# AtharvBhat/otters

Measured on AMD Instinct MI355X. Metric: GB/s scanned + queries/sec, exact cosine top-10 over 10M x 768 f32 rows per GPU, higher is better.
Workload: dtype f32; 1 GPU; 10000000x768 f32 VecStore per GPU, single query, Metric::Cosine, take(10); rows_per_gpu=10000000, dim=768, k=10, nq=1, processes=1

## Files before the change

### otters_amd/csrc/ott_exact.hip

```cpp
#include <atomic>

#include "ott_internal.h"
#include "ott_prune.h"
#include "ott_i8_check.h"
#include "ott_exact_dev.h"

namespace ott {

constexpr int KC = 32;
constexpr int WAVES = 4;
constexpr int STAGE_FLOATS = 64 * KC;
constexpr int EXACT_SMEM = WAVES * STAGE_FLOATS * 4;
constexpr int DUMP_QCAP = 128;
constexpr int EXACT_SMEM_DUMP = EXACT_SMEM + WAVES * DUMP_QCAP * 12;
constexpr int PQ_CAP = 128;
constexpr int PQ_WORDS = 10;
constexpr int QD_WORDS = (int)(OTT_QEMB_MAX / KC) * 12;
constexpr int EXACT_SMEM_PRUNE = EXACT_SMEM + WAVES * PQ_CAP * PQ_WORDS * 4 + QD_WORDS * 4;
constexpr int Q8_WORDS = (int)((OTT_QEMB_MAX + 127) / 128) * 32;
constexpr int EXACT_SMEM_CHECK = EXACT_SMEM_PRUNE + Q8_WORDS * 4;
#ifdef OTT_SK4_DECODE_F32
constexpr bool SK4_INT = false;
#else
constexpr bool SK4_INT = true;
#endif
constexpr int SK_MAXW = (int)OTT_SKETCH1_MAX_WORDS;
constexpr int SK3_MAXST = (int)OTT_SKETCH_MAX_WORDS / 3;
constexpr int SK3_XP = ((int)OTT_SKETCH_MAX_WORDS + 2 + 3) / 4 - 8;
#ifndef OTT_X_BLOCKS_PER_CU
#define OTT_X_BLOCKS_PER_CU 2
#endif
constexpr int BLOCKS_PER_CU = OTT_X_BLOCKS_PER_CU;
constexpr int SMALL_RING = 8;
constexpr uint32_t SMALL_QMAX = 2048;
[[maybe_unused]] constexpr int EXACT_SMEM_SMALL = SMALL_RING * STAGE_FLOATS * 4 + SMALL_QMAX * 4;

__device__ __forceinline__ void exact_glds16(const char* sbase, uint32_t voff, uint32_t lds_addr) {
    uint32_t keep;
    lds_addr = (uint32_t)__builtin_amdgcn_readfirstlane((int)lds_addr);
    asm volatile(
        "s_nop 4\n\t"
        "s_mov_b32 %0, m0\n\t"
        "s_mov_b32 m0, %3\n\t"
        "s_nop 0\n\t"
        "global_load_lds_dwordx4 %1, %2\n\t"
        "s_mov_b32 m0, %0"
        : "=&s"(keep)
        : "v"(voff), "s"(sbase), "s"(lds_addr)
        : "memory");
}


template <int MK, int NQ, int E, bool PERQ, bool DUMP = false, bool SMALL = false, bool BLK = (E > 1), bool I8 = false, bool PRUNE = false, int SK = 0, bool SEED = false,
          bool CHK = false>
__global__ __launch_bounds__(SMALL ? 64 : 256) void exact_kernel(ExactParams p) {
    static_assert(!CHK || (SK == 5 && !SEED && E == 1), "the int8 check is the gated head launch's, one list entry per lane");
    static_assert(!I8 || (NQ == 1 && MK == MK_DOT && !PERQ && !DUMP && !SMALL), "the int8 sweep takes one query, cosine / dot, merged");
    static_assert(!PRUNE || (NQ == 1 && MK == MK_DOT && !PERQ && !DUMP && !SMALL && !I8), "the pruned sweep takes one query, cosine / dot, merged");
    static_assert((SK == 0 || PRUNE) && (SK == 0 || SK == 1 || SK == 3 || SK == 4 || SK == 5), "the sketch is the pruned sweep's: none, one, three or four bits per dim (5: four with a head)");
    constexpr bool HD = SK == 5;
    constexpr bool SK4 = SK == 4 || SK == 5;
    static_assert(!HD || SK4_INT, "the head form decodes by integer dot products only");
    static_assert(!SEED || (HD && E == 1), "the estimate pass is the head form's, one list entry per lane");
    extern __shared__ __attribute__((aligned(16))) float smem[];
    const int lane = threadIdx.x & 63;
    const int wave = __builtin_amdgcn_readfirstlane(threadIdx.x >> 6);
    constexpr int BW = SMALL ? 1 : WAVES;
    float* st = SMALL ? smem : smem + wave * STAGE_FLOATS;
    float* sQ = smem + SMALL_RING * STAGE_FLOATS;
    constexpr int NL = PERQ ? NQ : 1;
    constexpr int KS = 64 * E;

    WaveList<E> L[NL];
    uint64_t tk[NL];
    uint32_t tq[NL];
    bool fresh[NL];
#pragma unroll
    for (int i = 0; i < NL; i++) {
        wl_init(L[i]);
        tk[i] = 0;
        tq[i] = 0xFFFFFFFFu;
        fresh[i] = true;
    }

    const bool take_max = p.take_max != 0;
    const uint32_t nq_here = (p.nq_total - p.q0) < (uint32_t)NQ ? (p.nq_total - p.q0) : (uint32_t)NQ;
    typedef __attribute__((address_space(4))) const float* CF32;
    typedef __attribute__((address_space(4))) const uint32_t* CU32;
    typedef __attribute__((address_space(4))) const ott_run* CRUN;
    typedef __attribute__((address_space(4))) const char* CCH;
    const CCH karg = (CCH)__builtin_amdgcn_kernarg_segment_ptr();
    const CF32 Q = p.embedded ? (CF32)(karg + __builtin_offsetof(ExactParams, qemb)) : (CF32)(p.queries + (size_t)p.q0 * p.dimq);
    const CU32 tile_prefix = p.embedded ? (CU32)(karg + __builtin_offsetof(ExactParams, eprefix)) : (CU32)p.tile_prefix;
    const CRUN runs = p.embedded ? (CRUN)(karg + __builtin_offsetof(ExactParams, eruns)) : (CRUN)p.runs;
    float qinv[NQ];
#pragma unroll
    for (int q = 0; q < NQ; q++) qinv[q] = (uint32_t)q < nq_here ? (p.embedded ? p.eqinv : p.qinv[p.q0 + q]) : 0.0f;
    uint32_t dgate[NQ];
#pragma unroll
    for (int q = 0; q < NQ; q++) dgate[q] = (DUMP && p.dump_gate != nullptr && (uint32_t)q < nq_here) ? p.dump_gate[p.q0 + q] : 0u;
    uint64_t* dq_key = reinterpret_cast<uint64_t*>(smem + WAVES * STAGE_FLOATS) + wave * DUMP_QCAP;
    uint32_t* dq_q = reinterpret_cast<uint32_t*>(smem + WAVES * STAGE_FLOATS + WAVES * DUMP_QCAP * 2) + wave * DUMP_QCAP;
    uint32_t dqn = 0;
    auto dq_flush = [&]() {
        if (dqn == 0) return;
        wave_sync();
        unsigned long long base = 0;
        if (lane == 0) base = atomicAdd(p.dump_cursor, (unsigned long long)dqn);
        base = rl64(base, 0);
        for (uint32_t i = lane; i < dqn; i += 64) {
            const uint64_t at = base + i;
            if (at < p.dump_cap) {
                p.dump_keys[at] = dq_key[i];
                p.dump_q[at] = dq_q[i];
            }
        }
        wave_sync();
        dqn = 0;
    };

    if constexpr (SMALL) {
        for (uint32_t i = threadIdx.x; i < p.dimq; i += 64 * BW) sQ[i] = Q[i];
        __syncthreads();
    }
    const uint32_t gw = blockIdx.x * BW + wave, nw = gridDim.x * BW;
    const int sw = (lane >> 1) & 7;
    const uint32_t nstages = (p.ld + KC - 1) / KC;
    [[maybe_unused]] uint32_t* qd = reinterpret_cast<uint32_t*>(smem + WAVES * STAGE_FLOATS + WAVES * PQ_CAP * PQ_WORDS);
    [[maybe_unused]] uint32_t* q8w = qd + QD_WORDS;
    [[maybe_unused]] const uint32_t ld8w = ((p.dim + 127u) & ~127u) >> 2;
    if constexpr (CHK) {
        const float pf8 = p.metric == OTT_METRIC_COSINE ? qinv[0] : 1.0f;
        const float inv_sq = __fdiv_rn(1.0f, p.i8_qscale);
        const uint32_t nw8 = ld8w < (uint32_t)Q8_WORDS ? ld8w : (uint32_t)Q8_WORDS;
        for (uint32_t i = threadIdx.x; i < nw8; i += 64 * BW) {
            float q4[4];
#pragma unroll
            for (int j = 0; j < 4; j++) q4[j] = (4 * i + j < p.dim) ? Q[4 * i + j] : 0.0f;
            q8w[i] = i8_quant_word(q4, pf8, inv_sq);
        }
    }
    if constexpr (SK4 && SK4_INT) {
        const uint32_t nqs = nstages < (uint32_t)(QD_WORDS / 12) ? nstages : (uint32_t)(QD_WORDS / 12);
        for (uint32_t i = threadIdx.x; i < nqs * 4; i += 64 * BW) {
            float q8[8];
#pragma unroll
            for (int j = 0; j < 8; j++) q8[j] = (8 * i + j < p.dim) ? Q[8 * i + j] : 0.0f;
            uint32_t d3[3];
            prune_quant_word(q8, p.prune_qinv_scale, d3);
#pragma unroll
            for (int d = 0; d < 3; d++) qd[(i >> 2) * 12 + d * 4 + (i & 3)] = d3[d];
        }
        __syncthreads();
    }
    const int lrow = lane >> 3;
    const int lslot = lane & 7;
    const uint32_t lsl4 = ((uint32_t)lslot * 4 < p.ld) ? (uint32_t)lslot * 4 : 0u;

    const uint32_t pstage = HD ? 0u : p.prune_stage;
    const uint32_t s_end = PRUNE ? pstage : nstages;
    uint32_t theta = 0;
    if constexpr (PRUNE && !SEED) {
        if (p.prune_seed[0] >= p.k) theta = ord_of(reinterpret_cast<const ott_hit*>(p.prune_seed + 8)[p.k - 1].score, take_max);
    }
    float* pq = smem + WAVES * STAGE_FLOATS + wave * (PQ_CAP * PQ_WORDS);
    uint32_t* pq_row = reinterpret_cast<uint32_t*>(pq + 9 * PQ_CAP);
    uint32_t pq_head = 0, pq_n = 0;
    uint32_t tails_done = 0;
    auto pq_finish = [&](uint32_t n) {
        wave_sync();
        const bool valid = (uint32_t)lane < n;
        const uint32_t e = (pq_head + (valid ? (uint32_t)lane : 0u)) & (PQ_CAP - 1);
        float acc[8];
#pragma unroll
        for (int l = 0; l < 8; l++) acc[l] = pq[l * PQ_CAP + e];
        const float vinv = pq[8 * PQ_CAP + e];
        const uint32_t my_row = pq_row[e];
        float tail = 0.0f;
        const float* rp[8];
        bool rok[8];
#pragma unroll
        for (int m = 0; m < 8; m++) {
            const uint32_t i = 8 * m + lrow;
            rok[m] = i < n;
            rp[m] = p.rows + (uint64_t)pq_row[(pq_head + (rok[m] ? i : 0u)) & (PQ_CAP - 1)] * p.ld + lsl4;
        }
        v4f R[8];
        auto load_stage = [&](uint32_t s) {
            const uint32_t soff = (s * KC + lslot * 4 < p.ld) ? s * KC : 0u;
#pragma unroll
            for (int m = 0; m < 8; m++) R[m] = __builtin_nontemporal_load(reinterpret_cast<const v4f*>(rp[m] + soff));
        };
        load_stage(pstage);
        for (uint32_t s = pstage; s < nstages; s++) {
            const bool cok = s * KC + lslot * 4 < p.ld;
#pragma unroll
            for (int m = 0; m < 8; m++) {
                const int row = 8 * m + lrow;
                const bool ok = rok[m] & cok;
                const v4f v = R[m];
                *reinterpret_cast<float4*>(st + row * KC + ((lslot ^ ((row >> 1) & 7)) << 2)) =
                    make_float4(ok ? v.x : 0.f, ok ? v.y : 0.f, ok ? v.z : 0.f, ok ? v.w : 0.f);
            }
            wave_sync();
            if (s + 1 < nstages) load_stage(s + 1);
#pragma unroll
            for (int j = 0; j < KC / 8; j++) {
                const uint32_t col = s * KC + 8 * j;
                if (col < p.dim) {
                    const float4 a = *reinterpret_cast<const float4*>(st + lane * KC + (((2 * j) ^ sw) << 2));
                    const float4 b = *reinterpret_cast<const float4*>(st + lane * KC + (((2 * j + 1) ^ sw) << 2));
                    const float x[8] = {a.x, a.y, a.z, a.w, b.x, b.y, b.z, b.w};
                    if (col + 8 <= p.dim) {
#pragma unroll
                        for (int l = 0; l < 8; l++) acc[l] = __fadd_rn(acc[l], exact_term<MK>(Q[col + l], x[l]));
                    } else {
                        const uint32_t nt = p.dim - col;
#pragma unroll
                        for (int l = 0; l < 7; l++)
                            if ((uint32_t)l < nt) tail = __fadd_rn(tail, exact_term<MK>(Q[col + l], x[l]));
                    }
                }
            }
            wave_sync();
        }
        float sc = __fadd_rn(reduce8(acc, p.reduce), tail);
        if (p.metric == OTT_METRIC_COSINE) sc = __fmul_rn(__fmul_rn(sc, qinv[0]), vinv);
        const bool pass = valid && !(sc != sc) && cmp_holds(sc, p.cmp, p.thr);
        const uint64_t key = ((uint64_t)ord_of(sc, take_max) << 32) | (uint32_t)(~(my_row + p.tie_off));
        if (fresh[0]) {
            wl_fill_sorted(L[0], tk[0], tq[0], p.k, pass, key, p.q0, lane, p.tie_sh);
            fresh[0] = false;
        } else if constexpr (!BLK) {
            wl_offer(L[0], tk[0], tq[0], p.k, pass, key, p.q0, lane, p.tie_sh);
        } else {
            wl_offer_block(L[0], tk[0], tq[0], p.k, pass, key, p.q0, lane, p.tie_sh);
        }
        pq_head = (pq_head + n) & (PQ_CAP - 1);
        pq_n -= n;
        tails_done += n;
    };
    [[maybe_unused]] uint32_t queued = 0;
    [[maybe_unused]] auto pq_refine = [&](uint32_t n, uint32_t gate) __attribute__((always_inline)) -> uint32_t {
        typedef uint32_t v4u __attribute__((ext_vector_type(4)));
        wave_sync();
        const bool valid = (uint32_t)lane < n;
        const uint32_t e = (pq_head + (valid ? (uint32_t)lane : 0u)) & (PQ_CAP - 1);
        const float vinv = pq[8 * PQ_CAP + e];
        const uint32_t my_row = pq_row[e];
        const float sv = p.i8_scale[my_row];
        const uint32_t fl = p.flag[my_row];
        const uint32_t* rp[8];
#pragma unroll
        for (int m = 0; m < 8; m++) {
            const uint32_t i = 8 * m + lrow;
            rp[m] = reinterpret_cast<const uint32_t*>(p.chk_plane) + (uint64_t)pq_row[(pq_head + (i < n ? i : 0u)) & (PQ_CAP - 1)] * ld8w + (uint32_t)lslot * 4;
        }
        v4f R[8];
        auto load_stage = [&](uint32_t s) {
#pragma unroll
            for (int m = 0; m < 8; m++) R[m] = __builtin_nontemporal_load(reinterpret_cast<const v4f*>(rp[m] + s * KC));
        };
        const uint32_t nst8 = ld8w / KC;
        int iacc[2] = {0, 0};
        load_stage(0);
        for (uint32_t s = 0; s < nst8; s++) {
#pragma unroll
            for (int m = 0; m < 8; m++) {
                const int row = 8 * m + lrow;
                const v4f v = R[m];
                *reinterpret_cast<float4*>(st + row * KC + ((lslot ^ ((row >> 1) & 7)) << 2)) = make_float4(v.x, v.y, v.z, v.w);
            }
            wave_sync();
            if (s + 1 < nst8) load_stage(s + 1);
#pragma unroll
            for (int j = 0; j < KC / 8; j++) {
                const float4 a = *reinterpret_cast<const float4*>(st + lane * KC + (((2 * j) ^ sw) << 2));
                const float4 b = *reinterpret_cast<const float4*>(st + lane * KC + (((2 * j + 1) ^ sw) << 2));
                const int x[8] = {__float_as_int(a.x), __float_as_int(a.y), __float_as_int(a.z), __float_as_int(a.w),
                                  __float_as_int(b.x), __float_as_int(b.y), __float_as_int(b.z), __float_as_int(b.w)};
                const v4u* qp = reinterpret_cast<const v4u*>(q8w + s * KC + 8 * j);
                const v4u q0 = qp[0], q1 = qp[1];
#pragma unroll
                for (int l = 0; l < 4; l++) {
                    iacc[0] = __builtin_amdgcn_sdot4(x[l], (int)q0[l], iacc[0], false);
                    iacc[1] = __builtin_amdgcn_sdot4(x[4 + l], (int)q1[l], iacc[1], false);
                }
            }
            wave_sync();
        }
        const float approx = i8_approx_score(iacc[0] + iacc[1], i8_row_factor(p.metric == OTT_METRIC_COSINE, vinv, sv, p.i8_qscale));
        const bool stay = valid && !i8_check_drops(approx, p.chk_eps, take_max, gate, (fl & 5u) != 0);
        const uint64_t km = __ballot(stay);
        if (stay) {
            const uint32_t at = (pq_head + (uint32_t)__popcll(km & ((1ull << lane) - 1ull))) & (PQ_CAP - 1);
            pq[8 * PQ_CAP + at] = vinv;
            pq_row[at] = my_row;
        }
        return (uint32_t)__popcll(km);
    };
    [[maybe_unused]] auto pq_drain = [&](uint32_t n, uint32_t gate) __attribute__((always_inline)) {
        const uint32_t stay = gate != 0 ? pq_refine(n, gate) : n;
        if (stay) pq_finish(stay);
        pq_head = (pq_head + (n - stay)) & (PQ_CAP - 1);
        pq_n -= n - stay;
    };

    if constexpr (HD) {
        typedef uint32_t v4u __attribute__((ext_vector_type(4)));
        const uint32_t np = p.sk_pitch >> 2;
        auto locate = [&](uint32_t t, uint64_t& row0, uint32_t& cnt, uint64_t& vm) {
            uint32_t lo = 0, hi = p.n_runs;
            while (hi - lo > 1) {
                uint32_t mid = (lo + hi) >> 1;
                if (tile_prefix[mid] <= t) lo = mid;
                else hi = mid;
            }
            const uint64_t rs = runs[lo].start, rc = runs[lo].count;
            const uint64_t off = (uint64_t)(t - tile_prefix[lo]) * 64;
            row0 = rs + off;
            cnt = (rc - off) < 64 ? (uint32_t)(rc - off) : 64u;
            const uint64_t r = row0 + lane;
            bool valid = (uint32_t)lane < cnt;
            if (p.row_mask != nullptr && valid && r < p.row_mask_bits) valid = (p.row_mask[r >> 6] >> (r & 63)) & 1;
            vm = __ballot(valid);
        };
        auto next_tile = [&](uint32_t t, uint64_t& row0, uint32_t& cnt, uint64_t& vm) -> uint32_t {
            for (; t < p.n_tiles; t += nw) {
                locate(t, row0, cnt, vm);
                if (vm != 0) break;
            }
            return t;
        };
        v4f R[8];
        v4u hc = {0u, 0u, 0u, 0u};
        float hrho = __builtin_inff(), hinv = 0.0f;
        auto load_line = [&](uint64_t row0, uint32_t cnt, uint32_t f) {
            const uint32_t pc = (8 * f + (uint32_t)lslot < np) ? 8 * f + (uint32_t)lslot : np - 1;
            const uint32_t* lb = p.prune_sketch + row0 * (uint64_t)p.sk_pitch + 4 * pc;
#pragma unroll
            for (int m = 0; m < 8; m++) {
                const uint32_t row = 8 * m + lrow;
                R[m] = __builtin_nontemporal_load(reinterpret_cast<const v4f*>(lb + (row < cnt ? row : cnt - 1) * p.sk_pitch));
            }
        };
        auto load_head = [&](uint64_t row0, uint32_t cnt) {
            const uint64_t r = row0 + ((uint32_t)lane < cnt ? (uint32_t)lane : cnt - 1);
            hc = __builtin_nontemporal_load(reinterpret_cast<const v4u*>(p.prune_head_codes) + r);
            hrho = __builtin_nontemporal_load(p.prune_head_rho + r);
            hinv = __builtin_nontemporal_load(p.inv + r);
        };
        uint64_t row0 = 0, vm = 0;
        uint32_t cnt = 0;
        uint32_t t = next_tile(gw, row0, cnt, vm);
        bool pf = false;
        while (t < p.n_tiles) {
            uint32_t gate = theta;
            const uint32_t own = (uint32_t)(tk[0] >> 32);
            if (own > gate) gate = own;
            const uint64_t my_row = row0 + lane;
            const bool valid = (vm >> lane) & 1;
            uint64_t row0n = 0, vmn = 0;
            uint32_t cntn = 0;
            const uint32_t tn = next_tile(t + nw, row0n, cntn, vmn);
            bool keep = valid;
            float vinv = 0.0f;
            if (SEED || gate != 0) {
                if (!pf) {
                    load_line(row0, cnt, 0);
                    load_head(row0, cnt);
                }
                const v4u c0 = hc;
                const float rho_all = hrho;
                vinv = hinv;
                pf = false;
                int K0 = 0, K1 = 0, K2 = 0;
                float sk_a = 0.0f;
                for (uint32_t f = 0; 8 * f < np; f++) {
#pragma unroll
                    for (int m = 0; m < 8; m++) {
                        const int row = 8 * m + lrow;
                        const v4f v = R[m];
                        *reinterpret_cast<float4*>(st + row * KC + ((lslot ^ ((row >> 1) & 7)) << 2)) = make_float4(v.x, v.y, v.z, v.w);
                    }
                    wave_sync();
                    if (8 * (f + 1) < np) {
                        load_line(row0, cnt, f + 1);
                    } else if (tn < p.n_tiles) {
                        load_line(row0n, cntn, 0);
                        load_head(row0n, cntn);
                        pf = true;
                    }
                    for (uint32_t j = 0; j < 8 && 8 * f + j < np; j++) {
                        const float4 w4 = *reinterpret_cast<const float4*>(st + lane * KC + (((int)j ^ sw) << 2));
                        const uint32_t piece = 8 * f + j;
                        if (piece == 0) {
                            sk_a = w4.x;
                            continue;
                        }
                        const uint32_t sj = p.sk_stage0 + piece - 1u;
                        if (sj < nstages) {
                            const uint32_t w[4] = {__float_as_uint(w4.x), __float_as_uint(w4.y), __float_as_uint(w4.z), __float_as_uint(w4.w)};
                            const v4u* dp = reinterpret_cast<const v4u*>(qd + sj * 12);
                            const v4u d0 = dp[0], d1 = dp[1], d2 = dp[2];
#pragma unroll
                            for (int i = 0; i < 4; i++) {
                                K0 = __builtin_amdgcn_sdot8((int)w[i], (int)d0[i], K0, false);
                                K1 = __builtin_amdgcn_sdot8((int)w[i], (int)d1[i], K1, false);
                                K2 = __builtin_amdgcn_sdot8((int)w[i], (int)d2[i], K2, false);
                            }
                        }
                    }
                    wave_sync();
                }
                {
                    const v4u* dp = reinterpret_cast<const v4u*>(qd);
                    const v4u d0 = dp[0], d1 = dp[1], d2 = dp[2];
#pragma unroll
                    for (int i = 0; i < 4; i++) {
                        K0 = __builtin_amdgcn_sdot8((int)c0[i], (int)d0[i], K0, false);
                        K1 = __builtin_amdgcn_sdot8((int)c0[i], (int)d1[i], K1, false);
                        K2 = __builtin_amdgcn_sdot8((int)c0[i], (int)d2[i], K2, false);
                    }
                }
                if constexpr (SEED) {
                    const int K = 2 * (256 * K2 + 16 * K1 + K0) + p.prune_qsum;
                    const float est = prune_score_est_sketchq(vinv, sk_a, rho_all, K, p.prune_qscale, qinv[0], p.metric == OTT_METRIC_COSINE);
                    const bool offer = valid && est - est == 0.0f;
                    const uint64_t key = ((uint64_t)ord_of(est, take_max) << 32) | (uint32_t)(~(uint32_t)my_row);
                    if (fresh[0]) {
                        wl_fill_sorted(L[0], tk[0], tq[0], p.seed_keep, offer, key, p.q0, lane, 0u);
                        fresh[0] = false;
                    } else {
                        wl_offer(L[0], tk[0], tq[0], p.seed_keep, offer, key, p.q0, lane, 0u);
                    }
                    keep = false;
                } else if (valid) {
                    const float zero[8] = {0.f, 0.f, 0.f, 0.f, 0.f, 0.f, 0.f, 0.f};
                    const int K = 2 * (256 * K2 + 16 * K1 + K0) + p.prune_qsum;
                    const float b = prune_score_bound_sketchq(zero, vinv, sk_a, rho_all, K, p.prune_qscale, p.dim, p.prune_qt, p.prune_qe1, p.prune_qn, qinv[0],
                                                              p.metric == OTT_METRIC_COSINE, take_max);
                    keep = !(b == b && ord_of(b, take_max) < gate);
                }
            } else if (valid) {
                vinv = p.inv[my_row];
            }
            const uint64_t km = SEED ? 0ull : __ballot(keep);
            if (!SEED && keep) {
                const uint32_t at = (pq_head + pq_n + (uint32_t)__popcll(km & ((1ull << lane) - 1ull))) & (PQ_CAP - 1);
#pragma unroll
                for (int l = 0; l < 8; l++) pq[l * PQ_CAP + at] = 0.0f;
                pq[8 * PQ_CAP + at] = vinv;
                pq_row[at] = (uint32_t)my_row;
            }
            pq_n += (uint32_t)__popcll(km);
            if constexpr (CHK) queued += (uint32_t)__popcll(km);
            if (!SEED && pq_n >= 64) {
                if constexpr (CHK) pq_drain(64, gate);
                else pq_finish(64);
                if (pf) {
                    load_line(row0n, cntn, 0);
                    load_head(row0n, cntn);
                }
            }
            t = tn;
            row0 = row0n;
            cnt = cntn;
            vm = vmn;
        }
        if constexpr (SEED) {
            const bool have = (uint32_t)lane < p.seed_keep && L[0].key[0] != 0ull;
            const uint64_t hm = __ballot(have);
            if (have) {
                const uint32_t r = ~(uint32_t)L[0].key[0];
                const uint32_t at = (uint32_t)__popcll(hm & ((1ull << lane) - 1ull));
#pragma unroll
                for (int l = 0; l < 8; l++) pq[l * PQ_CAP + at] = 0.0f;
                pq[8 * PQ_CAP + at] = p.inv[r];
                pq_row[at] = r;
            }
            pq_n = (uint32_t)__popcll(hm);
            wl_init(L[0]);
            tk[0] = 0;
            tq[0] = 0xFFFFFFFFu;
            fresh[0] = true;
        }
    } else
    for (uint32_t t = gw; t < p.n_tiles; t += nw) {
        uint32_t lo = 0, hi = p.n_runs;
        while (hi - lo > 1) {
            uint32_t mid = (lo + hi) >> 1;
            if (tile_prefix[mid] <= t) lo = mid;
            else hi = mid;
        }
        ott_run run;
        run.start = runs[lo].start;
        run.count = runs[lo].count;
        const uint64_t off = (uint64_t)(t - tile_prefix[lo]) * 64;
        const uint64_t row0 = run.start + off;
        const uint32_t cnt = (run.count - off) < 64 ? (uint32_t)(run.count - off) : 64u;
        const uint64_t my_row = row0 + lane;
        bool valid = (uint32_t)lane < cnt;
        if (p.row_mask != nullptr && valid && my_row < p.row_mask_bits)
            valid = (p.row_mask[my_row >> 6] >> (my_row & 63)) & 1;
        if (__ballot(valid) == 0) continue;

        float vinv = 0.0f;
        if ((PRUNE || p.metric == OTT_METRIC_COSINE) && valid) vinv = p.inv[my_row];
        float vsq = 0.0f;
        typedef uint32_t v4u __attribute__((ext_vector_type(4)));
        [[maybe_unused]] uint32_t skl[2 + SK_MAXW];
        [[maybe_unused]] uint32_t gate3 = 0;
        if constexpr (SK >= 3) {
            gate3 = theta;
            const uint32_t own = (uint32_t)(tk[0] >> 32);
            if (own > gate3) gate3 = own;
        }
        if constexpr (SK == 1) {
#pragma unroll
            for (int i = 0; i < 2 + SK_MAXW; i++) skl[i] = 0u;
            skl[1] = 0x7F800000u;
            if (valid) {
                const v4u* sp = reinterpret_cast<const v4u*>(p.prune_sketch + my_row * (uint64_t)p.sk_pitch);
                const v4u l0 = __builtin_nontemporal_load(sp);
                v4u l1 = {0u, 0u, 0u, 0u}, l2 = {0u, 0u, 0u, 0u};
                if (p.sk_pitch > 4) l1 = __builtin_nontemporal_load(sp + 1);
                if (p.sk_pitch > 8) l2 = __builtin_nontemporal_load(sp + 2);
                skl[0] = l0.x; skl[1] = l0.y; skl[2] = l0.z; skl[3] = l0.w;
                skl[4] = l1.x; skl[5] = l1.y; skl[6] = l1.z; skl[7] = l1.w;
                skl[8] = l2.x; skl[9] = l2.y; skl[10] = l2.z; skl[11] = l2.w;
            }
        }
        float i8_rf = 0.0f;
        bool i8_forced = false;
        if constexpr (I8) {
            if (valid) {
                i8_rf = ((p.metric == OTT_METRIC_COSINE ? vinv : 1.0f) * p.i8_scale[my_row]) * p.i8_qscale;
                i8_forced = (p.flag[my_row] & 5u) != 0;
            }
        }
        int iacc[2] = {0, 0};
        float acc[NQ][8];
        float tail[NQ];
#pragma unroll
        for (int q = 0; q < NQ; q++) {
            tail[q] = 0.0f;
#pragma unroll
            for (int l = 0; l < 8; l++) acc[q][l] = 0.0f;
        }

        v4f R[8];
        const float* rp[8];
        bool rok[8];
        const uint32_t lds_ring = (uint32_t)(uintptr_t)(__attribute__((address_space(3))) void*)st;
        const char* dma_base = reinterpret_cast<const char*>(p.rows + row0 * (uint64_t)p.ld);
        uint32_t dma_row[8];
        if constexpr (SMALL) {
#pragma unroll
            for (int m = 0; m < 8; m++) {
                const uint32_t row = 8 * m + lrow;
                dma_row[m] = (row < cnt ? row : cnt - 1) * p.ld;
            }
        } else {
#pragma unroll
            for (int m = 0; m < 8; m++) {
                const uint32_t row = 8 * m + lrow;
                rok[m] = row < cnt;
                rp[m] = p.rows + (row0 + (rok[m] ? row : cnt - 1)) * (uint64_t)p.ld + lsl4;
            }
        }
        auto dma_stage = [&](uint32_t s) {
            const uint32_t slot_e = lslot ^ (lrow >> 1);
#pragma unroll
            for (int m = 0; m < 8; m++) {
                const uint32_t col = s * KC + ((m & 1) ? (slot_e ^ 4) : slot_e) * 4;
                exact_glds16(dma_base, (dma_row[m] + (col < p.ld ? col : 0u)) * 4u,
                             lds_ring + (uint32_t)((s % SMALL_RING) * STAGE_FLOATS * 4 + m * 1024));
            }
        };
        auto load_stage = [&](uint32_t s) {
            const uint32_t soff = (s * KC + lslot * 4 < p.ld) ? s * KC : 0u;
#pragma unroll
            for (int m = 0; m < 8; m++) {
                R[m] = __builtin_nontemporal_load(reinterpret_cast<const v4f*>(rp[m] + soff));
            }
        };

        auto load_line = [&](uint32_t f) {
            const uint32_t np = p.sk_pitch >> 2;
            const uint32_t pc = (8 * f + (uint32_t)lslot < np) ? 8 * f + (uint32_t)lslot : np - 1;
            const uint32_t* lb = p.prune_sketch + row0 * (uint64_t)p.sk_pitch + 4 * pc;
#pragma unroll
            for (int m = 0; m < 8; m++) {
                const uint32_t row = 8 * m + lrow;
                R[m] = __builtin_nontemporal_load(reinterpret_cast<const v4f*>(lb + (row < cnt ? row : cnt - 1) * p.sk_pitch));
            }
        };

        if constexpr (SMALL) {
            for (uint32_t s = 0; s < (uint32_t)(SMALL_RING - 1) && s < nstages; s++) dma_stage(s);
        } else {
            load_stage(0);
        }
        for (uint32_t s = 0; s < s_end; s++) {
            const float* sst = st;
            if constexpr (SMALL) {
                const uint32_t later = (nstages - 1 - s) < (uint32_t)(SMALL_RING - 2) ? (nstages - 1 - s) : (uint32_t)(SMALL_RING - 2);
                switch (later) {
                    case 0: asm volatile("s_waitcnt vmcnt(0)" ::: "memory"); break;
                    case 1: asm volatile("s_waitcnt vmcnt(8)" ::: "memory"); break;
                    case 2: asm volatile("s_waitcnt vmcnt(16)" ::: "memory"); break;
                    case 3: asm volatile("s_waitcnt vmcnt(24)" ::: "memory"); break;
// ... 134 lines not shown
                                    for (int b = 0; b < 32; b++) {
                                        const int code = (int)(w[b >> 3] << (28 - 4 * (b & 7))) >> 28;
                                        D = fmaf((float)(2 * code + 1), Q[sj * KC + b], D);
                                    }
                                }
                            }
                        }
                        wave_sync();
                    }
                    if (valid) {
                        float b;
                        if constexpr (SK4_INT) {
                            const int K = 2 * (256 * K2 + 16 * K1 + K0) + p.prune_qsum;
                            b = prune_score_bound_sketchq(acc[0], vinv, sk_a, sk_rho, K, p.prune_qscale, p.dim, p.prune_qt, p.prune_qe1, p.prune_qn, qinv[0],
                                                          p.metric == OTT_METRIC_COSINE, take_max);
                        } else {
                            b = prune_score_bound_sketchb(acc[0], vinv, sk_a, sk_rho, D, 15.0, p.prune_stage * KC, p.dim, p.prune_qt, p.prune_q1,
                                                          p.prune_qn, qinv[0], p.metric == OTT_METRIC_COSINE, take_max);
                        }
                        keep = !(b == b && ord_of(b, take_max) < gate);
                    }
                }
            } else if constexpr (SK == 3) {
                if (gate != 0) {
                    v4f X[SK3_XP];
#pragma unroll
                    for (int i = 0; i < SK3_XP; i++) X[i] = R[7];
                    const uint32_t np = p.sk_pitch >> 2;
                    if (np > 8) {
                        const uint64_t lr = row0 + ((uint32_t)lane < cnt ? (uint32_t)lane : cnt - 1);
                        const v4f* sp = reinterpret_cast<const v4f*>(p.prune_sketch + lr * (uint64_t)p.sk_pitch);
#pragma unroll
                        for (int i = 0; i < SK3_XP; i++) X[i] = __builtin_nontemporal_load(sp + ((uint32_t)(8 + i) < np ? (uint32_t)(8 + i) : np - 1));
                    }
                    auto word = [&](int k) -> uint32_t {
                        const v4f v = (k >> 2) < 8 ? R[(k >> 2) & 7] : X[((k >> 2) - 8) % SK3_XP];
                        return __float_as_uint(v[k & 3]);
                    };
                    float D = 0.0f;
#pragma unroll
                    for (int j = 0; j < SK3_MAXST; j++) {
                        const uint32_t sj = p.sk_stage0 + (uint32_t)j;
                        if (sj >= p.prune_stage && sj < nstages) {
                            const uint32_t w[3] = {word(2 + 3 * j), word(3 + 3 * j), word(4 + 3 * j)};
#pragma unroll
                            for (int b = 0; b < 32; b++) {
                                const int pos = 3 * b, lo = pos & 31;
                                uint32_t x = w[pos >> 5] >> lo;
                                if (lo + 3 > 32) x |= w[(pos >> 5) + 1] << (32 - lo);
                                const int code = (int)(x << 29) >> 29;
                                D = fmaf((float)(2 * code + 1), Q[sj * KC + b], D);
                            }
                        }
                    }
                    if (valid) {
                        const float b = prune_score_bound_sketchb(acc[0], vinv, __uint_as_float(word(0)), __uint_as_float(word(1)), D, 7.0, p.prune_stage * KC,
                                                                  p.dim, p.prune_qt, p.prune_q1, p.prune_qn, qinv[0], p.metric == OTT_METRIC_COSINE, take_max);
                        keep = !(b == b && ord_of(b, take_max) < gate);
                    }
                }
            } else if constexpr (SK == 1) {
                if (gate != 0) {
                    float D = 0.0f;
#pragma unroll
                    for (int j = 0; j < SK_MAXW; j++) {
                        const uint32_t sj = p.sk_stage0 + (uint32_t)j;
                        if (sj >= p.prune_stage && sj < nstages) {
                            const uint32_t w = skl[2 + j];
#pragma unroll
                            for (int b = 0; b < 32; b++) {
                                const float sg = __uint_as_float(((w << (31 - b)) & 0x80000000u) | 0x3F800000u);
                                D = fmaf(sg, Q[sj * KC + b], D);
                            }
                        }
                    }
                    if (valid) {
                        const float b = prune_score_bound_sketch(acc[0], vinv, __uint_as_float(skl[0]), __uint_as_float(skl[1]), D, p.prune_stage * KC,
                                                                 p.dim, p.prune_qt, p.prune_q1, p.prune_qn, qinv[0], p.metric == OTT_METRIC_COSINE, take_max);
                        keep = !(b == b && ord_of(b, take_max) < gate);
                    }
                }
            } else if (valid && gate != 0) {
                const float b = prune_score_bound(acc[0], vsq, vinv, p.prune_stage * KC, p.dim, p.prune_qt, p.prune_qn, qinv[0],
                                                  p.metric == OTT_METRIC_COSINE, take_max);
                keep = !(b == b && ord_of(b, take_max) < gate);
            }
            const uint64_t km = __ballot(keep);
            if (keep) {
                const uint32_t at = (pq_head + pq_n + (uint32_t)__popcll(km & ((1ull << lane) - 1ull))) & (PQ_CAP - 1);
#pragma unroll
                for (int l = 0; l < 8; l++) pq[l * PQ_CAP + at] = acc[0][l];
                pq[8 * PQ_CAP + at] = vinv;
                pq_row[at] = (uint32_t)my_row;
            }
            pq_n += (uint32_t)__popcll(km);
            if (pq_n >= 64) pq_finish(64);
            continue;
        }

#pragma unroll
        for (int q = 0; q < NQ; q++) {
            if ((uint32_t)q < nq_here) {
                float s = __fadd_rn(reduce8(acc[q], p.reduce), tail[q]);
                if (p.metric == OTT_METRIC_COSINE) s = __fmul_rn(__fmul_rn(s, qinv[q]), vinv);
                bool pass = valid && !(s != s) && cmp_holds(s, p.cmp, p.thr);
                if constexpr (I8) {
                    s = (float)(iacc[0] + iacc[1]) * i8_rf;
                    pass = valid && !(s != s) && cmp_holds(s, p.cmp, p.thr);
                    if (i8_forced) {
                        s = take_max ? __builtin_inff() : -__builtin_inff();
                        pass = valid;
                    }
                }
                const uint64_t key = ((uint64_t)ord_of(p.flat ? 0.0f : s, take_max) << 32) | (uint32_t)(~((uint32_t)my_row + p.tie_off));
                if (DUMP) {
                    const bool keep = pass && (uint32_t)(key >> 32) >= dgate[q];
                    const uint64_t m = __ballot(keep);
                    if (m) {
                        const uint32_t c = (uint32_t)__popcll(m);
                        if (dqn + c > DUMP_QCAP) dq_flush();
                        if (keep) {
                            const uint32_t at = dqn + (uint32_t)__popcll(m & ((1ull << lane) - 1ull));
                            dq_key[at] = key;
                            dq_q[at] = p.q0 + q;
                        }
                        dqn += c;
                    }
                } else {
                    constexpr int li_max = NL - 1;
                    const int li = PERQ ? q : 0;
                    const int lx = li <= li_max ? li : 0;
                    if (fresh[lx]) {
                        wl_fill_sorted(L[lx], tk[lx], tq[lx], p.k, pass, key, p.q0 + q, lane, p.tie_sh);
                        fresh[lx] = false;
                        continue;
                    }
                    if constexpr (!BLK) wl_offer(L[lx], tk[lx], tq[lx], p.k, pass, key, p.q0 + q, lane, p.tie_sh);
                    else wl_offer_block(L[lx], tk[lx], tq[lx], p.k, pass, key, p.q0 + q, lane, p.tie_sh);
                }
            }
        }
    }

    if constexpr (CHK) {
        if (pq_n) {
            const uint32_t own = (uint32_t)(tk[0] >> 32);
            pq_drain(pq_n, own > theta ? own : theta);
        }
        if (p.prune_tails != nullptr && lane == 0) {
            if (queued != 0) atomicAdd(p.prune_tails, (unsigned long long)queued);
            if (tails_done != 0) atomicAdd(p.prune_tails + 1, (unsigned long long)tails_done);
        }
    } else if constexpr (PRUNE) {
        if (pq_n) pq_finish(pq_n);
        if (p.prune_tails != nullptr && tails_done != 0 && lane == 0) atomicAdd(p.prune_tails, (unsigned long long)tails_done);
    }
    if (DUMP) {
        dq_flush();
        return;
    }
    Cand* sl = reinterpret_cast<Cand*>(smem);
#pragma unroll
    for (int i = 0; i < NL; i++) {
        __syncthreads();
        if (wave > 0) {
#pragma unroll
            for (int e = 0; e < E; e++) {
                Cand c;
                c.key = L[i].key[e];
                c.q = L[i].q[e];
                c.pad = 0;
                sl[(wave - 1) * KS + e * 64 + lane] = c;
            }
        }
        __syncthreads();
        if (wave == 0) {
            for (int w = 0; w < BW - 1; w++) {
#pragma unroll
                for (int e = 0; e < E; e++) {
                    const uint32_t ppos = e * 64 + lane;
                    const Cand c = sl[w * KS + ppos];
                    const bool real = ppos < p.k && c.key != 0;
                    if constexpr (!BLK) {
                        wl_offer(L[i], tk[i], tq[i], p.k, real, c.key, c.q, lane, p.tie_sh);
                    } else {
                        const bool pass = real && before(c.key, c.q, tk[i], tq[i], p.tie_sh);
                        if (__popcll(__ballot(pass)) < WL_BLOCK_MIN) {
                            wl_offer(L[i], tk[i], tq[i], p.k, pass, c.key, c.q, lane, p.tie_sh);
                        } else {
                            wl_merge_sorted(L[i], real ? c.key : 0ull, real ? c.q : 0xFFFFFFFFu, lane, p.tie_sh);
                            wl_tau(L[i], p.k, tk[i], tq[i]);
                        }
                    }
                }
            }
            Cand* dst;
            if (PERQ) dst = p.lists + ((size_t)(p.q0 + i) * gridDim.x + blockIdx.x) * p.list_stride;
            else dst = p.lists + (size_t)blockIdx.x * p.list_stride;
            if (!PERQ || (uint32_t)i < nq_here) {
#pragma unroll
                for (int e = 0; e < E; e++) {
                    Cand c;
                    c.key = L[i].key[e];
                    c.q = L[i].q[e];
                    c.pad = 0;
                    dst[e * 64 + lane] = c;
                }
            }
        }
    }
}

constexpr int R8_WAVES = 8;
constexpr int R8_UNROLL = 12;
constexpr int R8_SMEM_MAX = (8 * (int)SMALL_QMAX + 8 * 64 + 64) * 4;

template <int MK, int E, int NQ, bool PERQ>
__global__ __launch_bounds__(64 * R8_WAVES) void exact_rows8_kernel(ExactParams p) {
    extern __shared__ __attribute__((aligned(16))) float smem[];
    float* sQ = smem;
    float* sS = smem + (size_t)NQ * p.dimq;
    uint32_t* sV = reinterpret_cast<uint32_t*>(sS + NQ * 64);
    const int lane = threadIdx.x & 63;
    const int wave = __builtin_amdgcn_readfirstlane(threadIdx.x >> 6);
    const int grp = lane >> 3, c = lane & 7;
    typedef __attribute__((address_space(4))) const float* CF32;
    typedef __attribute__((address_space(4))) const uint32_t* CU32;
    typedef __attribute__((address_space(4))) const ott_run* CRUN;
    typedef __attribute__((address_space(4))) const char* CCH;
    const CCH karg = (CCH)__builtin_amdgcn_kernarg_segment_ptr();
    const CF32 Q = p.embedded ? (CF32)(karg + __builtin_offsetof(ExactParams, qemb)) : (CF32)(p.queries + (size_t)p.q0 * p.dimq);
    const CU32 tile_prefix = p.embedded ? (CU32)(karg + __builtin_offsetof(ExactParams, eprefix)) : (CU32)p.tile_prefix;
    const CRUN runs = p.embedded ? (CRUN)(karg + __builtin_offsetof(ExactParams, eruns)) : (CRUN)p.runs;
    const uint32_t nq_here = (p.nq_total - p.q0) < (uint32_t)NQ ? (p.nq_total - p.q0) : (uint32_t)NQ;
    float qinv[NQ];
#pragma unroll
    for (int q = 0; q < NQ; q++) qinv[q] = (uint32_t)q < nq_here ? (p.embedded ? p.eqinv : p.qinv[p.q0 + q]) : 0.0f;
    for (uint32_t i = threadIdx.x; i < (uint32_t)NQ * p.dimq; i += 64 * R8_WAVES) sQ[i] = Q[i];

    const uint32_t t = blockIdx.x;
    uint32_t lo = 0, hi = p.n_runs;
    while (hi - lo > 1) {
        const uint32_t mid = (lo + hi) >> 1;
        if (tile_prefix[mid] <= t) lo = mid;
        else hi = mid;
    }
    const uint64_t rstart = runs[lo].start, rcount = runs[lo].count;
    const uint64_t off = (uint64_t)(t - tile_prefix[lo]) * 64;
    const uint64_t row0 = rstart + off;
    const uint32_t cnt = (rcount - off) < 64 ? (uint32_t)(rcount - off) : 64u;
    const uint32_t lrow = 8u * (uint32_t)wave + (uint32_t)grp;
    bool valid = lrow < cnt;
    const uint64_t my_row = row0 + (valid ? lrow : cnt - 1);
    if (p.row_mask != nullptr && valid && my_row < p.row_mask_bits) valid = (p.row_mask[my_row >> 6] >> (my_row & 63)) & 1;
    const float* rp = p.rows + my_row * (uint64_t)p.ld;
    float vinv = 0.0f;
    if (p.metric == OTT_METRIC_COSINE) vinv = p.inv[my_row];
    __syncthreads();

    const uint32_t full = p.dim >> 3;
    float acc[NQ];
#pragma unroll
    for (int q = 0; q < NQ; q++) acc[q] = 0.0f;
    auto step = [&](uint32_t jj, float xv) {
#pragma unroll
        for (int q = 0; q < NQ; q++) {
            const float qv = sQ[(uint32_t)q * p.dimq + 8 * jj + c];
            acc[q] = __fadd_rn(acc[q], exact_term<MK>(qv, xv));
        }
    };
    uint32_t j = 0;
    for (; j + R8_UNROLL <= full; j += R8_UNROLL) {
        float x[R8_UNROLL];
#pragma unroll
        for (int u = 0; u < R8_UNROLL; u++) x[u] = rp[8 * (j + u) + c];
#pragma unroll
        for (int u = 0; u < R8_UNROLL; u++) step(j + u, x[u]);
    }
    for (; j < full; j++) step(j, rp[8 * j + c]);
    float tail[NQ];
#pragma unroll
    for (int q = 0; q < NQ; q++) tail[q] = 0.0f;
    const uint32_t nt = p.dim & 7u;
    for (uint32_t l = 0; l < nt; l++) {
        const float xv = rp[8 * full + l];
#pragma unroll
        for (int q = 0; q < NQ; q++) {
            const float qv = sQ[(uint32_t)q * p.dimq + 8 * full + l];
            tail[q] = __fadd_rn(tail[q], exact_term<MK>(qv, xv));
        }
    }
#pragma unroll
    for (int q = 0; q < NQ; q++) {
        float sum;
        if (p.reduce == OTT_REDUCE_SEQ4) {
            const int b = lane & ~7;
            float l8[8];
#pragma unroll
            for (int i = 0; i < 8; i++) l8[i] = __shfl(acc[q], b + i);
            sum = reduce8(l8, OTT_REDUCE_SEQ4);
        } else {
            const float s1 = __fadd_rn(acc[q], __shfl_xor(acc[q], 4));
            const float s2 = __fadd_rn(s1, __shfl_xor(s1, 2));
            sum = __fadd_rn(s2, __shfl_xor(s2, 1));
        }
        float sc = __fadd_rn(sum, tail[q]);
        if (p.metric == OTT_METRIC_COSINE) sc = __fmul_rn(__fmul_rn(sc, qinv[q]), vinv);
// ... 812 lines not shown
```

### otters_amd/csrc/ott_exact_plan.h

```cpp
#pragma once
#include <stddef.h>

#include "../../include/otters_hip.h"

namespace ott {

constexpr uint32_t OTT_QEMB_MAX = 896;
constexpr uint32_t OTT_SKETCH_MAX_WORDS = 54;
constexpr uint32_t OTT_SKETCH1_MAX_WORDS = 10;
constexpr uint32_t OTT_SKETCH4_MAX_WORDS = 108;

inline int list_E(uint64_t k) { return k <= 64 ? 1 : k <= 128 ? 2 : k <= 256 ? 4 : 8; }
inline uint32_t list_stride(int E) { return 64u * (uint32_t)E; }

enum ExactRoute {
    EXACT_LISTS,
    EXACT_SORT,
    EXACT_REFUSED,
};
inline ExactRoute lists_or_sort(uint64_t k_eff, uint32_t nq, uint64_t rows_scored, int large_k_from, bool fetch) {
    if (k_eff > 512) return fetch ? EXACT_SORT : EXACT_REFUSED;
    const uint64_t pairs = rows_scored * nq;
    const uint64_t from = large_k_from > 0 ? (uint64_t)large_k_from : ((nq == 1 || pairs <= (1ull << 19)) ? 512u : 128u);
    return k_eff > from && fetch && pairs <= (1ull << 28) ? EXACT_SORT : EXACT_LISTS;
}

inline bool small_variant_fits(uint32_t dimq, uint64_t tiles) { return dimq <= 2048 && tiles <= 1024; }
inline uint32_t exact_variant(int exact_small, uint32_t nq, bool perq, int E, uint32_t dimq, uint32_t n_tiles) {
    const bool fits = E <= 2 && small_variant_fits(dimq, n_tiles);
    if (exact_small == 1) return fits && nq == 1 && !perq ? 1u : 0u;
    if (exact_small == 2 || exact_small < 0) return fits && nq <= 16 ? 2u : 0u;
    return 0u;
}

inline uint32_t pow2_at_least(uint32_t v) {
    uint32_t p = 1;
    while (p < v) p <<= 1;
    return p;
}
inline uint32_t queries_per_pass(uint32_t nq, int E, uint32_t variant) {
    if (E >= 4) return 1;
    const uint32_t most = variant == 2 ? 8u : 4u, p2 = pow2_at_least(nq);
    return p2 < most ? p2 : most;
}
inline bool exact_lean(uint32_t nq, uint32_t dimq, size_t n_runs) { return nq == 1 && dimq <= OTT_QEMB_MAX && n_runs <= 2; }

struct ExactPlan {
    int E;
    uint32_t KS;
    uint32_t variant;
    uint32_t tile;
    uint32_t passes;
    int grid;
    bool lean;
};
inline ExactPlan exact_plan(uint64_t k_eff, uint32_t nq, bool perq, uint32_t dimq, uint32_t n_tiles, size_t n_runs, int exact_small, int stream_grid) {
    ExactPlan x;
    x.E = list_E(k_eff);
    x.KS = list_stride(x.E);
    x.variant = exact_variant(exact_small, nq, perq, x.E, dimq, n_tiles);
    x.tile = queries_per_pass(nq, x.E, x.variant);
    x.passes = (nq + x.tile - 1) / x.tile;
    x.grid = x.variant ? (int)n_tiles : stream_grid;
    x.lean = exact_lean(nq, dimq, n_runs);
    return x;
}
inline size_t exact_n_lists(const ExactPlan& x, uint32_t nq, bool perq, bool pruned, int gridA, int gridB) {
    return pruned ? (size_t)(gridA + gridB) : perq ? (size_t)nq * x.grid : (size_t)x.passes * x.grid;
}

#ifndef OTT_X_SEED_DIV
#define OTT_X_SEED_DIV 32
#endif
struct SketchState {
    bool present;
    bool covers;
    uint32_t bits, words, stage0;
};
struct PruneIn {
    uint32_t dim, ld, metric;
    bool perq, lean, flat;
    uint32_t variant;
    int exact_prune, exact_sketch;
    SketchState sk;
    uint64_t rows_scored;
    int E;
};
struct PrunePlan {
    uint32_t c;
    bool sketch;
    uint64_t seed;
};
inline PrunePlan prune_plan(const PruneIn& in) {
    const PrunePlan off{0, false, 0};
    if (!(in.lean && !in.perq && in.variant == 0 && !in.flat && in.exact_prune != 0 && (in.metric == OTT_METRIC_COSINE || in.metric == OTT_METRIC_DOT)))
        return off;
    const uint32_t nst = (in.ld + 31) / 32;
    uint32_t c = nst * 7 / 8;
    while (c > 0 && c * 32 > in.dim - in.dim % 8) c--;
    bool sketch = false;
    if (in.exact_sketch != 0 && in.sk.present && in.sk.covers &&
        in.sk.words <= (in.sk.bits == 4 ? OTT_SKETCH4_MAX_WORDS : in.sk.bits == 3 ? OTT_SKETCH_MAX_WORDS : OTT_SKETCH1_MAX_WORDS)) {
        const uint32_t cs = in.sk.stage0;
        if (cs >= 1 && cs < nst && cs * 32 <= in.dim - in.dim % 8) {
            c = cs;
            sketch = true;
        }
    }
    const bool worth = in.exact_prune == 1 || (nst >= 8 && in.rows_scored >= (1ull << 20));
    if (!(worth && c >= 1 && c < nst)) return off;
    uint64_t seed = in.rows_scored / 10;
    if (sketch && in.sk.bits >= 3 && in.E == 1 && seed > 131072) seed = in.rows_scored / OTT_X_SEED_DIV > 131072 ? in.rows_scored / OTT_X_SEED_DIV : 131072;
    seed = (seed + 63) & ~63ull;
    if (seed < 64) seed = 64;
    return PrunePlan{c, sketch, seed};
}
inline bool prune_plan_needs_quant(const PruneIn& in, const PrunePlan& pp) { return pp.c != 0 && pp.sketch && in.sk.bits == 4; }
struct HeadState {
    bool present;
    bool covers;
    int option;
};
inline bool prune_plan_head(const PruneIn& in, const PrunePlan& pp, bool quant_ok, const HeadState& hd) {
    return prune_plan_needs_quant(in, pp) && quant_ok && hd.present && hd.covers && hd.option != 0 && in.E <= 4;
}
#ifndef OTT_X_I8_CHECK
#define OTT_X_I8_CHECK 1
#endif
struct I8CheckState {
    bool plane_ready;
    int option;
    bool eps_ok;
};
inline bool prune_plan_i8_check(const PruneIn& in, const PrunePlan& pp, bool head, const I8CheckState& ck) {
    return OTT_X_I8_CHECK != 0 && pp.c != 0 && head && in.E == 1 && ck.plane_ready && ck.option != 0 && ck.eps_ok;
}
#ifndef OTT_X_SEED_EST
#define OTT_X_SEED_EST 1
#endif
#ifndef OTT_X_SEED_EST_DIV
#define OTT_X_SEED_EST_DIV 0
#endif
#ifndef OTT_X_SEED_KEEP
#define OTT_X_SEED_KEEP 0
#endif
constexpr uint64_t SEED_EST_MIN_ROWS = 131072;
constexpr uint32_t SEED_EST_KEEP_MAX = 16;
inline uint64_t prune_plan_seed_est(const PruneIn& in, const PrunePlan& pp, bool head, bool filtered) {
    if (!OTT_X_SEED_EST || !head || in.E != 1 || filtered || pp.c == 0 || in.rows_scored / 10 < SEED_EST_MIN_ROWS) return 0;
    uint64_t rows = pp.seed;
    if (OTT_X_SEED_EST_DIV > 0) {
        rows = (in.rows_scored / (uint64_t)(OTT_X_SEED_EST_DIV > 0 ? OTT_X_SEED_EST_DIV : 1) + 63) & ~63ull;
        if (rows < SEED_EST_MIN_ROWS) rows = SEED_EST_MIN_ROWS;
    }
    return rows;
}
inline uint32_t prune_seed_keep(uint64_t k) {
    if (OTT_X_SEED_KEEP > 0) return OTT_X_SEED_KEEP < 64 ? (uint32_t)OTT_X_SEED_KEEP : 64u;
    return k < SEED_EST_KEEP_MAX ? (uint32_t)k : SEED_EST_KEEP_MAX;
}
inline PrunePlan prune_plan_quant_refused(PruneIn in) {
    in.exact_sketch = 0;
    return prune_plan(in);
}

struct ExactResult {
    size_t cnt_pad;
    size_t bytes;
    size_t host_bytes;
};
inline ExactResult exact_result_layout(uint32_t groups, uint32_t KS) {
    const size_t cnt_pad = (((size_t)groups * sizeof(uint64_t)) + 63) & ~(size_t)63;
    const size_t bytes = cnt_pad + (size_t)groups * KS * sizeof(ott_hit);
    return ExactResult{cnt_pad, bytes, bytes + 8};
}

inline uint64_t exact_bytes_scanned(uint32_t passes, uint64_t rows_scored, uint32_t dim, uint32_t metric) {
    return (uint64_t)passes * rows_scored * ((uint64_t)dim * 4 + (metric == OTT_METRIC_COSINE ? 4 : 0));
}

}
```

Baseline: 40130 GB/s.

## Finish small pruned tail batches with multi-stage loads across idle row slots

Adds a finish path for batches of at most sixteen surviving rows in the head-sketch pruned sweep. Instead of spending a full 64-row stage per KC column block while most slots sit idle, each load round fetches several consecutive column stages for the one or two 8-row groups. The wave then walks those stages from LDS, which cuts the number of load/sync rounds per tail flush. It applies to the seed estimate pass and to small final drains, and adds index mapping complexity plus a new shared include for the stage and offer code.

```diff
diff --git a/otters_amd/csrc/ott_exact.hip b/otters_amd/csrc/ott_exact.hip
--- a/otters_amd/csrc/ott_exact.hip
+++ b/otters_amd/csrc/ott_exact.hip
@@ -3,6 +3,7 @@
 #include "ott_internal.h"
 #include "ott_prune.h"
 #include "ott_i8_check.h"
+#include "ott_finish_few.h"
 #include "ott_exact_dev.h"
 
 namespace ott {
@@ -31,6 +32,10 @@
 #define OTT_X_BLOCKS_PER_CU 2
 #endif
 constexpr int BLOCKS_PER_CU = OTT_X_BLOCKS_PER_CU;
+#ifndef OTT_X_FINISH_FEW
+#define OTT_X_FINISH_FEW 1
+#endif
+static_assert(KC == (int)FF_KC, "ott_finish_few.h walks stages of KC floats");
 constexpr int SMALL_RING = 8;
 constexpr uint32_t SMALL_QMAX = 2048;
 [[maybe_unused]] constexpr int EXACT_SMEM_SMALL = SMALL_RING * STAGE_FLOATS * 4 + SMALL_QMAX * 4;
@@ -62,6 +67,7 @@
     constexpr bool SK4 = SK == 4 || SK == 5;
     static_assert(!HD || SK4_INT, "the head form decodes by integer dot products only");
     static_assert(!SEED || (HD && E == 1), "the estimate pass is the head form's, one list entry per lane");
+    constexpr bool FEW = OTT_X_FINISH_FEW != 0 && HD && E == 1;
     extern __shared__ __attribute__((aligned(16))) float smem[];
     const int lane = threadIdx.x & 63;
     const int wave = __builtin_amdgcn_readfirstlane(threadIdx.x >> 6);
@@ -167,7 +173,7 @@
     uint32_t* pq_row = reinterpret_cast<uint32_t*>(pq + 9 * PQ_CAP);
     uint32_t pq_head = 0, pq_n = 0;
     uint32_t tails_done = 0;
-    auto pq_finish = [&](uint32_t n) {
+    [[maybe_unused]] auto pq_finish = [&](uint32_t n) {
         wave_sync();
         const bool valid = (uint32_t)lane < n;
         const uint32_t e = (pq_head + (valid ? (uint32_t)lane : 0u)) & (PQ_CAP - 1);
@@ -204,41 +210,76 @@
             }
             wave_sync();
             if (s + 1 < nstages) load_stage(s + 1);
-#pragma unroll
-            for (int j = 0; j < KC / 8; j++) {
-                const uint32_t col = s * KC + 8 * j;
-                if (col < p.dim) {
-                    const float4 a = *reinterpret_cast<const float4*>(st + lane * KC + (((2 * j) ^ sw) << 2));
-                    const float4 b = *reinterpret_cast<const float4*>(st + lane * KC + (((2 * j + 1) ^ sw) << 2));
-                    const float x[8] = {a.x, a.y, a.z, a.w, b.x, b.y, b.z, b.w};
-                    if (col + 8 <= p.dim) {
-#pragma unroll
-                        for (int l = 0; l < 8; l++) acc[l] = __fadd_rn(acc[l], exact_term<MK>(Q[col + l], x[l]));
-                    } else {
-                        const uint32_t nt = p.dim - col;
-#pragma unroll
-                        for (int l = 0; l < 7; l++)
-                            if ((uint32_t)l < nt) tail = __fadd_rn(tail, exact_term<MK>(Q[col + l], x[l]));
-                    }
-                }
+            {
+                const uint32_t cs_stage = s;
+                const float* cs_row = st + lane * KC;
+                const int cs_swz = sw;
+#include "ott_exact_finish_stage.inc"
             }
             wave_sync();
         }
-        float sc = __fadd_rn(reduce8(acc, p.reduce), tail);
-        if (p.metric == OTT_METRIC_COSINE) sc = __fmul_rn(__fmul_rn(sc, qinv[0]), vinv);
-        const bool pass = valid && !(sc != sc) && cmp_holds(sc, p.cmp, p.thr);
-        const uint64_t key = ((uint64_t)ord_of(sc, take_max) << 32) | (uint32_t)(~(my_row + p.tie_off));
-        if (fresh[0]) {
-            wl_fill_sorted(L[0], tk[0], tq[0], p.k, pass, key, p.q0, lane, p.tie_sh);
-            fresh[0] = false;
-        } else if constexpr (!BLK) {
-            wl_offer(L[0], tk[0], tq[0], p.k, pass, key, p.q0, lane, p.tie_sh);
+#include "ott_exact_finish_offer.inc"
+    };
+    [[maybe_unused]] auto pq_finish_few = [&](uint32_t n) __attribute__((always_inline)) {
+        wave_sync();
+        const bool valid = (uint32_t)lane < n;
+        const uint32_t e = (pq_head + (valid ? (uint32_t)lane : 0u)) & (PQ_CAP - 1);
+        float acc[8];
+#pragma unroll
+        for (int l = 0; l < 8; l++) acc[l] = pq[l * PQ_CAP + e];
+        const float vinv = pq[8 * PQ_CAP + e];
+        const uint32_t my_row = pq_row[e];
+        float tail = 0.0f;
+        const uint32_t S = ff_stages(n);
+        const float* rp[2];
+        bool rok[2];
+#pragma unroll
+        for (int g = 0; g < 2; g++) {
+            const uint32_t i = 8 * g + lrow;
+            rok[g] = i < n;
+            rp[g] = p.rows + (uint64_t)pq_row[(pq_head + (rok[g] ? i : 0u)) & (PQ_CAP - 1)] * p.ld + ff_slot_off((uint32_t)lslot, p.ld);
+        }
+        v4f R[8];
+        auto load_round = [&](uint32_t s0) __attribute__((always_inline)) {
+#pragma unroll
+            for (int m = 0; m < 8; m++) {
+                const uint32_t sc = ff_stage_clamp(s0 + ff_load_slab(m, n), nstages);
+                R[m] = __builtin_nontemporal_load(reinterpret_cast<const v4f*>((ff_load_group(m, n) ? rp[1] : rp[0]) + ff_col_off(sc, (uint32_t)lslot, p.ld)));
+            }
+        };
+        load_round(pstage);
+        const uint32_t li = (uint32_t)lane & (8u * ff_groups(n) - 1u);
+        for (uint32_t s0 = pstage; s0 < nstages; s0 += S) {
+#pragma unroll
+            for (int m = 0; m < 8; m++) {
+                const bool cok = ff_col_ok(s0 + ff_load_slab(m, n), (uint32_t)lslot, p.ld);
+                const bool ok = (ff_load_group(m, n) ? rok[1] : rok[0]) & cok;
+                const v4f v = R[m];
+                *reinterpret_cast<float4*>(st + ff_store_off(m, (uint32_t)lrow, (uint32_t)lslot)) =
+                    make_float4(ok ? v.x : 0.f, ok ? v.y : 0.f, ok ? v.z : 0.f, ok ? v.w : 0.f);
+            }
+            wave_sync();
+            if (s0 + S < nstages) load_round(s0 + S);
+            for (uint32_t sl = 0; sl < S && s0 + sl < nstages; sl++) {
+                const uint32_t brow = ff_read_off(li, n, sl, 0u) / KC;
+                const uint32_t cs_stage = s0 + sl;
+                const float* cs_row = st + brow * KC;
+                const int cs_swz = (int)((brow >> 1) & 7u);
+#include "ott_exact_finish_stage.inc"
+            }
+            wave_sync();
+        }
+#include "ott_exact_finish_offer.inc"
+    };
+    [[maybe_unused]] auto pq_finish_any = [&](uint32_t n) __attribute__((always_inline)) {
+        if constexpr (FEW && SEED) {
+            pq_finish_few(n);
+        } else if constexpr (FEW) {
+            if (n <= FF_MAX_ROWS) pq_finish_few(n);
+            else pq_finish(n);
         } else {
-            wl_offer_block(L[0], tk[0], tq[0], p.k, pass, key, p.q0, lane, p.tie_sh);
-        }
-        pq_head = (pq_head + n) & (PQ_CAP - 1);
-        pq_n -= n;
-        tails_done += n;
+            pq_finish(n);
+        }
     };
     [[maybe_unused]] uint32_t queued = 0;
     [[maybe_unused]] auto pq_refine = [&](uint32_t n, uint32_t gate) __attribute__((always_inline)) -> uint32_t {
@@ -301,7 +342,7 @@
     };
     [[maybe_unused]] auto pq_drain = [&](uint32_t n, uint32_t gate) __attribute__((always_inline)) {
         const uint32_t stay = gate != 0 ? pq_refine(n, gate) : n;
-        if (stay) pq_finish(stay);
+        if (stay) pq_finish_any(stay);
         pq_head = (pq_head + (n - stay)) & (PQ_CAP - 1);
         pq_n -= n - stay;
     };
@@ -457,7 +498,7 @@
             if constexpr (CHK) queued += (uint32_t)__popcll(km);
             if (!SEED && pq_n >= 64) {
                 if constexpr (CHK) pq_drain(64, gate);
-                else pq_finish(64);
+                else if constexpr (!SEED) pq_finish(64);
                 if (pf) {
                     load_line(row0n, cntn, 0);
                     load_head(row0n, cntn);
@@ -898,7 +939,10 @@
             if (tails_done != 0) atomicAdd(p.prune_tails + 1, (unsigned long long)tails_done);
         }
     } else if constexpr (PRUNE) {
-        if (pq_n) pq_finish(pq_n);
+        if (pq_n) {
+            if constexpr (FEW) pq_finish_any(pq_n);
+            else pq_finish(pq_n);
+        }
         if (p.prune_tails != nullptr && tails_done != 0 && lane == 0) atomicAdd(p.prune_tails, (unsigned long long)tails_done);
     }
     if (DUMP) {
diff --git a/otters_amd/csrc/ott_exact_finish_offer.inc b/otters_amd/csrc/ott_exact_finish_offer.inc
--- /dev/null
+++ b/otters_amd/csrc/ott_exact_finish_offer.inc
@@ -0,0 +1,15 @@
+float sc = __fadd_rn(reduce8(acc, p.reduce), tail);
+if (p.metric == OTT_METRIC_COSINE) sc = __fmul_rn(__fmul_rn(sc, qinv[0]), vinv);
+const bool pass = valid && !(sc != sc) && cmp_holds(sc, p.cmp, p.thr);
+const uint64_t key = ((uint64_t)ord_of(sc, take_max) << 32) | (uint32_t)(~(my_row + p.tie_off));
+if (fresh[0]) {
+    wl_fill_sorted(L[0], tk[0], tq[0], p.k, pass, key, p.q0, lane, p.tie_sh);
+    fresh[0] = false;
+} else if constexpr (!BLK) {
+    wl_offer(L[0], tk[0], tq[0], p.k, pass, key, p.q0, lane, p.tie_sh);
+} else {
+    wl_offer_block(L[0], tk[0], tq[0], p.k, pass, key, p.q0, lane, p.tie_sh);
+}
+pq_head = (pq_head + n) & (PQ_CAP - 1);
+pq_n -= n;
+tails_done += n;
diff --git a/otters_amd/csrc/ott_exact_finish_stage.inc b/otters_amd/csrc/ott_exact_finish_stage.inc
--- /dev/null
+++ b/otters_amd/csrc/ott_exact_finish_stage.inc
@@ -0,0 +1,18 @@
+#pragma unroll
+for (int j = 0; j < KC / 8; j++) {
+    const uint32_t col = cs_stage * KC + 8 * j;
+    if (col < p.dim) {
+        const float4 a = *reinterpret_cast<const float4*>(cs_row + (((2 * j) ^ cs_swz) << 2));
+        const float4 b = *reinterpret_cast<const float4*>(cs_row + (((2 * j + 1) ^ cs_swz) << 2));
+        const float x[8] = {a.x, a.y, a.z, a.w, b.x, b.y, b.z, b.w};
+        if (col + 8 <= p.dim) {
+#pragma unroll
+            for (int l = 0; l < 8; l++) acc[l] = __fadd_rn(acc[l], exact_term<MK>(Q[col + l], x[l]));
+        } else {
+            const uint32_t nt = p.dim - col;
+#pragma unroll
+            for (int l = 0; l < 7; l++)
+                if ((uint32_t)l < nt) tail = __fadd_rn(tail, exact_term<MK>(Q[col + l], x[l]));
+        }
+    }
+}
diff --git a/otters_amd/csrc/ott_exact_plan.h b/otters_amd/csrc/ott_exact_plan.h
--- a/otters_amd/csrc/ott_exact_plan.h
+++ b/otters_amd/csrc/ott_exact_plan.h
@@ -146,6 +146,7 @@
 #endif
 constexpr uint64_t SEED_EST_MIN_ROWS = 131072;
 constexpr uint32_t SEED_EST_KEEP_MAX = 16;
+static_assert(OTT_X_SEED_KEEP <= 16, "the estimate pass finishes at most sixteen rows per wave");
 inline uint64_t prune_plan_seed_est(const PruneIn& in, const PrunePlan& pp, bool head, bool filtered) {
     if (!OTT_X_SEED_EST || !head || in.E != 1 || filtered || pp.c == 0 || in.rows_scored / 10 < SEED_EST_MIN_ROWS) return 0;
     uint64_t rows = pp.seed;
diff --git a/otters_amd/csrc/ott_finish_few.h b/otters_amd/csrc/ott_finish_few.h
--- /dev/null
+++ b/otters_amd/csrc/ott_finish_few.h
@@ -0,0 +1,34 @@
+#pragma once
+#include <stdint.h>
+
+#if defined(__HIPCC__)
+#define OTT_FF_HD __host__ __device__
+#else
+#define OTT_FF_HD
+#endif
+
+namespace ott {
+
+constexpr uint32_t FF_MAX_ROWS = 16;
+constexpr uint32_t FF_KC = 32;
+
+OTT_FF_HD inline uint32_t ff_gshift(uint32_t n) { return n <= 8 ? 0u : 1u; }
+OTT_FF_HD inline uint32_t ff_groups(uint32_t n) { return 1u << ff_gshift(n); }
+OTT_FF_HD inline uint32_t ff_stages(uint32_t n) { return 8u >> ff_gshift(n); }
+OTT_FF_HD inline uint32_t ff_rounds(uint32_t n, uint32_t pstage, uint32_t nstages) {
+    const uint32_t S = ff_stages(n);
+    return nstages > pstage ? (nstages - pstage + S - 1) / S : 0u;
+}
+OTT_FF_HD inline uint32_t ff_load_slab(uint32_t m, uint32_t n) { return m >> ff_gshift(n); }
+OTT_FF_HD inline uint32_t ff_load_group(uint32_t m, uint32_t n) { return m & (ff_groups(n) - 1u); }
+OTT_FF_HD inline uint32_t ff_load_row(uint32_t m, uint32_t n, uint32_t lrow) { return 8u * ff_load_group(m, n) + lrow; }
+OTT_FF_HD inline uint32_t ff_stage(uint32_t n, uint32_t pstage, uint32_t r, uint32_t j) { return pstage + r * ff_stages(n) + j; }
+OTT_FF_HD inline uint32_t ff_stage_clamp(uint32_t s, uint32_t nstages) { return s < nstages ? s : nstages - 1u; }
+OTT_FF_HD inline uint32_t ff_slot_off(uint32_t lslot, uint32_t ld) { return lslot * 4u < ld ? lslot * 4u : 0u; }
+OTT_FF_HD inline uint32_t ff_col_off(uint32_t sc, uint32_t lslot, uint32_t ld) { return sc * FF_KC + lslot * 4u < ld ? sc * FF_KC : 0u; }
+OTT_FF_HD inline bool ff_col_ok(uint32_t s, uint32_t lslot, uint32_t ld) { return s * FF_KC + lslot * 4u < ld; }
+OTT_FF_HD inline uint32_t ff_buf_off(uint32_t brow, uint32_t slot) { return brow * FF_KC + ((slot ^ ((brow >> 1) & 7u)) << 2); }
+OTT_FF_HD inline uint32_t ff_store_off(uint32_t m, uint32_t lrow, uint32_t lslot) { return ff_buf_off(8u * m + lrow, lslot); }
+OTT_FF_HD inline uint32_t ff_read_off(uint32_t i, uint32_t n, uint32_t j, uint32_t slot) { return ff_buf_off(((j * 8u) << ff_gshift(n)) + i, slot); }
+
+}
```

New measurement: 40850 GB/s (median of 6 runs). 1.8% higher.
